# jcyk/gtos

Measured on AMD Instinct MI355X. Metric: graphs/sec training step (100-node AMR, batch 64), higher is better.
Workload: dtype bf16

## Files before the change

### gtos_amd/_lib.py

```python
import ctypes
import os
import threading

import torch

_HERE = os.path.dirname(os.path.abspath(__file__))
LIB_PATH = os.path.join(_HERE, "csrc", "libgtos_hip.so")
ABI_VERSION = 25

c_p, c_i, c_l, c_f, c_u64 = ctypes.c_void_p, ctypes.c_int, ctypes.c_int64, ctypes.c_float, ctypes.c_uint64

SIGNATURES = {
    "gtos_abi_version": [],
    "gtos_pathtrie_dev_workspace": [c_l, c_l, c_p],
    "gtos_pathtrie_dev_phase_a": [c_i, c_l, c_p, c_p, c_p, c_p, c_p, c_p, c_p, ctypes.c_size_t, c_p],
    "gtos_pathtrie_dev_phase_b": [c_l, c_l, c_i, c_i, c_i, c_i, c_p, c_p, c_p, c_p, c_p, ctypes.c_size_t, c_p],
    "gtos_relbatch_dev_workspace": [c_l, c_p],
    "gtos_relbatch_dev_phase_a": [c_p, c_p, c_p, ctypes.c_size_t, c_p],
    "gtos_relbatch_dev_phase_b": [c_p, c_l, c_p, c_p, ctypes.c_size_t, c_p],
    "gtos_relbatch_dev_all_count": [c_p, c_p, c_p, ctypes.c_size_t, c_p],
    "gtos_relbatch_dev_all_keys": [c_p, c_p, c_p, ctypes.c_size_t, c_p],
    "gtos_relbatch_dev_all_fill": [c_p, c_l, c_p, c_p, ctypes.c_size_t, c_p],
    "gtos_relindex_dev_workspace": [c_l, c_p],
    "gtos_relindex_dev_phase_a": [c_p, c_p, c_p, ctypes.c_size_t, c_p],
    "gtos_relindex_dev_phase_b": [c_p, c_l, c_p, c_p, ctypes.c_size_t, c_p],
    "gtos_gemm": [c_i, c_i, c_i, c_i, c_i, c_i, c_i, c_p, c_l, c_p, c_l, c_p, c_l, c_p, c_i, c_f, c_u64, c_i, c_i, c_p, c_l, c_p],
    "gtos_rel_attn_fwd": [c_i] * 7 + [c_p, c_l, c_p, c_l, c_p, c_l, c_p, c_p, c_p, c_p, c_f, c_f, c_u64, c_p, c_l, c_p, c_p, c_p],
    "gtos_rel_attn_bwd": [c_i] * 7 + [c_p, c_l, c_p, c_l, c_p, c_l, c_p, c_p, c_p, c_p, c_p, c_f, c_f, c_u64,
                                      c_p, c_l, c_p, c_p, c_p, c_l, c_p, c_p, c_l, c_p, c_l, c_p, c_l, c_p, c_l, c_p, c_p, c_p],
    "gtos_rel_attn_bwd_bank": [c_i] * 5 + [c_p, c_l, c_p, c_l, c_p, c_p, c_p, c_p, c_p, c_p, c_p, c_p, c_i, c_p, c_l, c_p, c_p],
    "gtos_ln_residual_fwd": [c_i, c_i, c_i, c_p, c_p, c_f, c_u64, c_p, c_p, c_f, c_p, c_p, c_p, c_p],
    "gtos_ln_residual_bwd": [c_i, c_i, c_i, c_p, c_p, c_p, c_f, c_u64, c_p, c_p, c_p, c_p, c_p, c_p, c_p, c_p],
    "gtos_ln_residual_fwd2": [c_i, c_i, c_i, c_i, c_i, c_p, c_p, c_f, c_u64, c_p, c_p, c_f, c_p, c_p, c_p, c_p, c_p],
    "gtos_ln_residual_bwd2": [c_i, c_i, c_i, c_i, c_i, c_p, c_p, c_p, c_p, c_f, c_u64, c_p, c_p, c_p, c_p, c_p, c_p, c_p, c_p],
    "gtos_relu_dropout_bwd": [c_i, c_l, c_p, c_p, c_f, c_p],
    "gtos_colsum": [c_i, c_i, c_i, c_l, c_p, c_p, c_p],
    "gtos_gru_cell_fwd": [c_i, c_i, c_i, c_p, c_p, c_p, c_p, c_l, c_p, c_p, c_f, c_u64, c_l, c_p],
    "gtos_gru_step_fwd": [c_i, c_i, c_p, c_l, c_i, c_p, c_p, c_p, c_p, c_p, c_p, c_p, c_p, c_p, c_p, c_p, c_p, c_i, c_p, c_l, c_p, c_p, c_p, c_l,
                          c_f, c_u64, c_l, c_p],
    "gtos_gru_step_bwd": [c_i, c_i, c_p, c_i, c_p, c_p, c_p, c_p, c_p, c_l, c_p, c_i, c_l, c_p, c_f, c_u64, c_l, c_p, c_i, c_p, c_p, c_p, c_i, c_p],
    "gtos_gru_step_bwd_fused": [c_i, c_i, c_p, c_i, c_p, c_p, c_p, c_p, c_p, c_l, c_p, c_i, c_l, c_p, c_f, c_u64, c_l, c_p, c_i, c_p, c_p, c_p, c_i,
# ... 115 lines not shown
```

### gtos_amd/csrc/gru_step.hip

```cpp
#include <cstdlib>
#include "common.h"

__attribute__((visibility("hidden"))) const void* gtos_zero_block();

#define GTOS_VMCNT(n) __builtin_amdgcn_s_waitcnt(0x0F70 | ((n) & 15) | (((n) >> 4) << 14))
#ifndef GTOS_RACE_DEMO
#define GTOS_VMCNT_LDS(n) __builtin_amdgcn_s_waitcnt(0x0070 | ((n) & 15) | (((n) >> 4) << 14))
#define GTOS_LGKM0() __builtin_amdgcn_s_waitcnt(0xc07f)
#else
#define GTOS_VMCNT_LDS(n) GTOS_VMCNT(n)
#define GTOS_LGKM0()
#endif

namespace {

constexpr int ROWB = 128, BK = 64, TM = 128, TC = 64, WROWS = 3 * TC;
constexpr int A_BYTES = TM * ROWB, B_BYTES = WROWS * ROWB;

__device__ __forceinline__ int swz(int row) { return ((row >> 1) & 7) ^ ((row >> 4) & 3); }
__device__ __forceinline__ int lds_off(int r, int c) { return r * ROWB + ((c ^ swz(r)) << 4); }

struct StepArgs {
    const bf16_t* x; int64_t ldx; int in_dim; const bf16_t* w_ih; const float* b_ih;
    const bf16_t* xg;
// ... 158 lines not shown
#pragma unroll
        for (int i = 0; i < 16; ++i) bhz[i] += t[i];
    }
    const float ks = a.p_drop > 0.f ? 1.f / (1.f - a.p_drop) : 1.f;
#pragma unroll
    for (int mt = 0; mt < 2; ++mt) {
        const int m = m0 + wave * 32 + mt * 16 + fr;
        if (m >= a.rows) continue;
        float xr[16], xz[16], xn[16], hp[16];
        if constexpr (HAS_X) {
            ldf16(a.b_ih + 2 * hs + cb, xn);
#pragma unroll
            for (int i = 0; i < 16; ++i) { xr[i] = 0.f; xz[i] = 0.f; xn[i] += acc[mt][8 + (i >> 2)][i & 3]; }
        } else if constexpr (MODE == 2) {
            const bf16_t* fp = a.gf + (int64_t)a.gf_idx[m] * 3 * hs + cb;
            const bf16_t* bp = a.gb + (int64_t)a.gb_idx[m] * 3 * hs + cb;
            float t[16];
            ld16(fp, xr); ld16(bp, t);
#pragma unroll
            for (int i = 0; i < 16; ++i) xr[i] += t[i];
            ld16(fp + hs, xz); ld16(bp + hs, t);
#pragma unroll
            for (int i = 0; i < 16; ++i) xz[i] += t[i];
            ld16(fp + 2 * hs, xn); ld16(bp + 2 * hs, t);
#pragma unroll
            for (int i = 0; i < 16; ++i) xn[i] += t[i];
            ldf16(a.b_ih + 2 * hs + cb, t);
#pragma unroll
            for (int i = 0; i < 16; ++i) xn[i] += t[i];
        } else {
            const bf16_t* xp = a.xg + (int64_t)m * 3 * hs + cb;
            ld16(xp, xr); ld16(xp + hs, xz); ld16(xp + 2 * hs, xn);
        }
        ld16(a.h_in + (int64_t)(a.h_idx ? a.h_idx[m] : m) * hs + cb, hp);
        float gr[16], gz[16], gn[16], hn[16], o[16];
#pragma unroll
        for (int i = 0; i < 16; ++i) {
            gr[i] = 1.f / (1.f + __expf(-(xr[i] + acc[mt][(i >> 2)][i & 3] + bhr[i])));
            gz[i] = 1.f / (1.f + __expf(-(xz[i] + acc[mt][4 + (i >> 2)][i & 3] + bhz[i])));
            hn[i] = acc[mt][GH * 4 + (i >> 2)][i & 3] + bhn[i];
            hn[i] = bf2f(f2bf(hn[i]));
            gn[i] = fast_tanh(xn[i] + gr[i] * hn[i]);
            o[i] = (1.f - gz[i]) * gn[i] + gz[i] * hp[i];
        }
        bf16_t* gp = a.gates + (int64_t)m * 4 * hs + cb;
        st16(gp, gr); st16(gp + hs, gz); st16(gp + 2 * hs, gn);
        st16(gp + 3 * hs, hn);
        bf16_t* hdst = m < a.n_out ? a.h_out + (int64_t)m * hs + cb
                                   : a.h_fin + (int64_t)(a.fin_idx ? a.fin_idx[m] : m) * a.ld_fin + cb;
        st16(hdst, o);
        if (a.y) {
            if (a.p_drop > 0.f) {
#pragma unroll
                for (int i = 0; i < 16; ++i)
                    o[i] = drop_keep(a.seed, (uint64_t)(a.drop_base + (int64_t)m * a.ldy + cb + i), a.p_drop) ? o[i] * ks : 0.f;
            }
            st16(a.y + (int64_t)m * a.ldy + cb, o);
        }
    }
}

template <int MODE>
__global__ __launch_bounds__(256, 2) void gru_step_fwd_kernel(StepArgs a) {
    if (a.p_drop > 0.f) a.seed = live_seed(a.seed);
    constexpr bool HAS_X = MODE == 1;
    constexpr int NG = HAS_X ? 4 : 3;
    constexpr int GH = HAS_X ? 3 : 2;
    __shared__ __attribute__((aligned(16))) char lds[A_BYTES + B_BYTES];
    char* As = lds;
    char* Bs = lds + A_BYTES;
    const int lane = threadIdx.x & 63, wave = __builtin_amdgcn_readfirstlane(threadIdx.x >> 6);
    const int fr = lane & 15, fq = lane >> 4;
    const int nC = a.hs / TC;
    const int xcd = blockIdx.x & 7, sq = blockIdx.x >> 3;
    const int m0 = ((sq / nC) * 8 + xcd) * TM, c0 = (sq % nC) * TC;
    if (m0 >= a.rows) return;
    const U128* Z = static_cast<const U128*>(a.zeros);

    f32x4_t acc[2][NG * 4];
#pragma unroll
    for (int i = 0; i < 2; ++i)
#pragma unroll
        for (int j = 0; j < NG * 4; ++j) acc[i][j] = f32x4_t{0.f, 0.f, 0.f, 0.f};

    if constexpr (HAS_X) {
        const RowSrc xs = row_src(a.x, a.ldx, a.rows, m0, wave, lane);
        const WSrc ws = w_src(a.in_dim, a.hs, c0, wave, lane);
        for (int k0 = 0; k0 < a.in_dim; k0 += BK) {
            dma_rows_at(xs, Z, k0, a.in_dim, As, wave);
            dma_weights_at(ws, a.w_ih, Z, k0, a.in_dim, Bs, wave);
            __syncthreads();
            mma_tile<NG, 2>(As, Bs, wave * 32, fr, fq, acc);
            __syncthreads();
        }
    }
    {
        const RowSrc hsrc = row_src(a.h_in, a.hs, a.rows, m0, wave, lane, a.h_idx);
        const WSrc ws = w_src(a.hs, a.hs, c0, wave, lane);
        for (int k0 = 0; k0 < a.hs; k0 += BK) {
            dma_rows_at(hsrc, Z, k0, a.hs, As, wave);
            dma_weights_at(ws, a.w_hh, Z, k0, a.hs, Bs, wave);
            __syncthreads();
            mma_tile<NG, GH>(As, Bs, wave * 32, fr, fq, acc);
            __syncthreads();
        }
    }

    step_cell<MODE>(a, acc, m0, c0, wave, fr, fq);
}


__global__ __launch_bounds__(512, 2) void gru_step_fwd_a2w3_kernel(StepArgs a) {
    constexpr int TMW = 256, AW = TMW * ROWB;
    if (a.p_drop > 0.f) a.seed = live_seed(a.seed);
    __shared__ __attribute__((aligned(16))) char sa0[AW];
    __shared__ __attribute__((aligned(16))) char sa1[AW];
    __shared__ __attribute__((aligned(16))) char sw0[B_BYTES];
    __shared__ __attribute__((aligned(16))) char sw1[B_BYTES];
    __shared__ __attribute__((aligned(16))) char sa2[AW];
    const int lane = threadIdx.x & 63, wave = __builtin_amdgcn_readfirstlane(threadIdx.x >> 6);
    const int fr = lane & 15, fq = lane >> 4;
    const int hs = a.hs, nC = hs / TC;
    const int xcd = blockIdx.x & 7, sq = blockIdx.x >> 3;
    const int m0 = ((sq / nC) * 8 + xcd) * TMW, c0 = (sq % nC) * TC;
    if (m0 >= a.rows) return;
    const int nkx = a.in_dim / BK, nk = nkx + hs / BK;
    uint32_t axo[4], aho[4], bxo[3], bho[3];
#pragma unroll
    for (int i = 0; i < 4; ++i) {
        const int rl = (i * 8 + wave) * 8 + (lane >> 3);
        const int r = min(m0 + rl, a.rows - 1) - m0;
        const uint32_t c = (uint32_t)(((lane & 7) ^ swz(rl)) << 4);
        axo[i] = (uint32_t)r * (uint32_t)(a.ldx * 2) + c;
        aho[i] = (uint32_t)r * (uint32_t)(hs * 2) + c;
    }
#pragma unroll
    for (int i = 0; i < 3; ++i) {
        const int rl = (i * 8 + wave) * 8 + (lane >> 3);
        const int g = rl >> 6, nt = (rl >> 4) & 3, q = (rl >> 2) & 3, e = rl & 3;
        const int wrow = g * hs + c0 + q * 16 + nt * 4 + e;
        const uint32_t c = (uint32_t)(((lane & 7) ^ swz(rl)) << 4);
        bxo[i] = (uint32_t)wrow * (uint32_t)(a.in_dim * 2) + c;
        bho[i] = (uint32_t)wrow * (uint32_t)(hs * 2) + c;
    }
    const char* Xb = reinterpret_cast<const char*>(a.x + (int64_t)m0 * a.ldx);
    const char* Hb = reinterpret_cast<const char*>(a.h_in + (int64_t)m0 * hs);
    const char* Wi = reinterpret_cast<const char*>(a.w_ih);
    const char* Wh = reinterpret_cast<const char*>(a.w_hh);

    f32x4_t acc[2][16];
#pragma unroll
    for (int i = 0; i < 2; ++i)
#pragma unroll
        for (int j = 0; j < 16; ++j) acc[i][j] = f32x4_t{0.f, 0.f, 0.f, 0.f};

#define GTOS_DMA1(src, dst)                                                                                                   \
    __builtin_amdgcn_global_load_lds((const __attribute__((address_space(1))) void*)(src),                                    \
                                     (__attribute__((address_space(3))) void*)(dst), 16, 0, 0)
#define GTOS_A2W3_DMA_A(slot, s_)                                                                                             \
    {                                                                                                                         \
        const int st_ = min((s_), nk - 1);                                                                                    \
        const bool px_ = st_ < nkx;                                                                                           \
        const char* ab_ = px_ ? Xb + st_ * ROWB : Hb + (st_ - nkx) * ROWB;                                                    \
        GTOS_DMA1(ab_ + (px_ ? axo[0] : aho[0]), (slot) + (0 * 8 + wave) * 1024);                                             \
        GTOS_DMA1(ab_ + (px_ ? axo[1] : aho[1]), (slot) + (1 * 8 + wave) * 1024);                                             \
        GTOS_DMA1(ab_ + (px_ ? axo[2] : aho[2]), (slot) + (2 * 8 + wave) * 1024);                                             \
        GTOS_DMA1(ab_ + (px_ ? axo[3] : aho[3]), (slot) + (3 * 8 + wave) * 1024);                                             \
    }
#define GTOS_A2W3_DMA_W(slot, s_)                                                                                             \
    {                                                                                                                         \
        const int st_ = min((s_), nk - 1);                                                                                    \
        const bool px_ = st_ < nkx;                                                                                           \
        const char* bb_ = px_ ? Wi + st_ * ROWB : Wh + (st_ - nkx) * ROWB;                                                    \
        GTOS_DMA1(bb_ + (px_ ? bxo[0] : bho[0]), (slot) + (0 * 8 + wave) * 1024);                                             \
        GTOS_DMA1(bb_ + (px_ ? bxo[1] : bho[1]), (slot) + (1 * 8 + wave) * 1024);                                             \
        GTOS_DMA1(bb_ + (px_ ? bxo[2] : bho[2]), (slot) + (2 * 8 + wave) * 1024);                                             \
    }
#define GTOS_A2W3_STEP(sa_, sw_, sa_n, sw_n, s_)                                                                              \
    {                                                                                                                         \
        GTOS_VMCNT_LDS(4);                                  \
        __builtin_amdgcn_s_barrier();                       \
        GTOS_A2W3_DMA_W(sw_n, (s_) + 1);                                                                                      \
        GTOS_A2W3_DMA_A(sa_n, (s_) + 2);                                                                                      \
        {                                                                                                                     \
            _Pragma("unroll") for (int ks = 0; ks < 2; ++ks) {                                                                \
                bf16x8_t fa[2], fb[12];                                                                                       \
                _Pragma("unroll") for (int mt = 0; mt < 2; ++mt)                                                              \
                    fa[mt] = *reinterpret_cast<const bf16x8_t*>((sa_) + lds_off(wave * 32 + mt * 16 + fr, ks * 4 + fq));      \
                _Pragma("unroll") for (int t = 0; t < 12; ++t)                                                                \
                    fb[t] = *reinterpret_cast<const bf16x8_t*>((sw_) + lds_off(t * 16 + fr, ks * 4 + fq));                    \
                _Pragma("unroll") for (int g = 0; g < 2; ++g)                                                                 \
                    _Pragma("unroll") for (int nt = 0; nt < 4; ++nt)                                                          \
                        _Pragma("unroll") for (int mt = 0; mt < 2; ++mt)                                                      \
                            acc[mt][g * 4 + nt] = __builtin_amdgcn_mfma_f32_16x16x32_bf16(fb[g * 4 + nt], fa[mt], acc[mt][g * 4 + nt], 0, 0, 0); \
                if ((s_) < nkx) {                                                                                             \
                    _Pragma("unroll") for (int nt = 0; nt < 4; ++nt)                                                          \
                        _Pragma("unroll") for (int mt = 0; mt < 2; ++mt)                                                      \
                            acc[mt][8 + nt] = __builtin_amdgcn_mfma_f32_16x16x32_bf16(fb[8 + nt], fa[mt], acc[mt][8 + nt], 0, 0, 0); \
                } else {                                                                                                      \
                    _Pragma("unroll") for (int nt = 0; nt < 4; ++nt)                                                          \
                        _Pragma("unroll") for (int mt = 0; mt < 2; ++mt)                                                      \
                            acc[mt][12 + nt] = __builtin_amdgcn_mfma_f32_16x16x32_bf16(fb[8 + nt], fa[mt], acc[mt][12 + nt], 0, 0, 0); \
                }                                                                                                             \
            }                                                                                                                 \
        }                                                                                                                     \
    }

    if (nk > 0) {
        GTOS_A2W3_DMA_A(sa0, 0);
        GTOS_A2W3_DMA_W(sw0, 0);
        GTOS_A2W3_DMA_A(sa1, 1);
    }
    for (int s = 0; s + 6 <= nk; s += 6) {
        GTOS_A2W3_STEP(sa0, sw0, sa2, sw1, s);
        GTOS_A2W3_STEP(sa1, sw1, sa0, sw0, s + 1);
        GTOS_A2W3_STEP(sa2, sw0, sa1, sw1, s + 2);
        GTOS_A2W3_STEP(sa0, sw1, sa2, sw0, s + 3);
        GTOS_A2W3_STEP(sa1, sw0, sa0, sw1, s + 4);
        GTOS_A2W3_STEP(sa2, sw1, sa1, sw0, s + 5);
    }
    GTOS_VMCNT(0);
#undef GTOS_A2W3_STEP
#undef GTOS_A2W3_DMA_W
#undef GTOS_A2W3_DMA_A
#undef GTOS_DMA1
    step_cell<1>(a, acc, m0, c0, wave, fr, fq);
}


struct Raw16 { uint4 a, b; };
__device__ __forceinline__ void unpack16(const Raw16& r, float (&v)[16]) {
    v[0] = lo_bf(r.a.x); v[1] = hi_bf(r.a.x); v[2] = lo_bf(r.a.y); v[3] = hi_bf(r.a.y);
    v[4] = lo_bf(r.a.z); v[5] = hi_bf(r.a.z); v[6] = lo_bf(r.a.w); v[7] = hi_bf(r.a.w);
    v[8] = lo_bf(r.b.x); v[9] = hi_bf(r.b.x); v[10] = lo_bf(r.b.y); v[11] = hi_bf(r.b.y);
    v[12] = lo_bf(r.b.z); v[13] = hi_bf(r.b.z); v[14] = lo_bf(r.b.w); v[15] = hi_bf(r.b.w);
}
__device__ __forceinline__ Raw16 ldraw16(const bf16_t* p) {
    Raw16 r;
    r.a = *reinterpret_cast<const uint4*>(p);
    r.b = *reinterpret_cast<const uint4*>(p + 8);
    return r;
}

constexpr int P_ROWS = 32;
constexpr int P_TM = 4 * P_ROWS;

template <int KT>
__global__ __launch_bounds__(256, 1) void gru_l1_fwd_persistent_kernel(StepArgs a, int n_workers) {
    extern __shared__ __attribute__((aligned(16))) char plds[];
    constexpr int HS = 64 * KT;
    constexpr int A_TILE = P_ROWS * ROWB;
    const int lane = threadIdx.x & 63, wave = __builtin_amdgcn_readfirstlane(threadIdx.x >> 6);
// ... 289 lines not shown
            __syncthreads();
#pragma unroll
            for (int ks = 0; ks < 2; ++ks) {
                bf16x8_t fa[2], fb[4];
#pragma unroll
                for (int mt = 0; mt < 2; ++mt) fa[mt] = *reinterpret_cast<const bf16x8_t*>(As + lds_off(wave * 32 + mt * 16 + fr, ks * 4 + fq));
#pragma unroll
                for (int nt = 0; nt < 4; ++nt) fb[nt] = *reinterpret_cast<const bf16x8_t*>(Bs + lds_off(nt * 16 + fr, ks * 4 + fq));
#pragma unroll
                for (int mt = 0; mt < 2; ++mt)
#pragma unroll
                    for (int nt = 0; nt < 4; ++nt)
                        acc[mt][nt] = __builtin_amdgcn_mfma_f32_16x16x32_bf16(fb[nt], fa[mt], acc[mt][nt], 0, 0, 0);
            }
            __syncthreads();
        }
    } else if (a.d4_prev && m0 < a.rows_prev) {
        kloop_a2<1, true>(a.d4_prev, 4 * (int64_t)hs, a.rows_prev, m0, a.wh_t, 3 * (int64_t)hs, c0, 1, hs, Z, As, lds_a1, Bs, acc, wave, lane);
    } else if (a.bias_part) {
        __syncthreads();
    }

    const int cb = c0 + fq * 16;
    const float ks = a.p_drop > 0.f ? 1.f / (1.f - a.p_drop) : 1.f;
#pragma unroll
    for (int mt = 0; mt < 2; ++mt) {
        const int m_raw = m0 + wave * 32 + mt * 16 + fr;
        const bool valid = m_raw < a.rows;
        const int m = valid ? m_raw : a.rows - 1;
        float gr[16], gz[16], gn[16], hn[16], hp[16], g[16];
        const bf16_t* gp = a.gates + (int64_t)m * 4 * hs + cb;
        ld16(gp, gr); ld16(gp + hs, gz); ld16(gp + 2 * hs, gn);
        ld16(gp + 3 * hs, hn);
        ld16(a.hprev + (int64_t)(a.hprev_idx ? a.hprev_idx[m] : m) * hs + cb, hp);
        float* dhp = static_cast<float*>(a.dh) + (int64_t)m * a.ld_dh + cb;
        bf16_t* dhb = static_cast<bf16_t*>(a.dh) + (int64_t)m * a.ld_dh + cb;
        if (a.sum_idx) {
            const int64_t sr = a.sum_idx[m];
            if (sr == a.zero_row) {
#pragma unroll
                for (int i = 0; i < 16; ++i) g[i] = 0.f;
            } else if (a.dh_bf16) ld16(static_cast<const bf16_t*>(a.dh_src) + sr * hs + cb, g);
            else ldf16(static_cast<const float*>(a.dh_src) + sr * hs + cb, g);
        } else if (a.dh_bf16) ld16(dhb, g); else ldf16(dhp, g);
#pragma unroll
        for (int i = 0; i < 16; ++i) g[i] += acc[mt][i >> 2][i & 3];
        if (a.dy) {
            float dyv[16];
            ld16(a.dy + (int64_t)m * a.ldy + cb, dyv);
#pragma unroll
            for (int i = 0; i < 16; ++i) {
                float t2 = dyv[i];
                if (a.p_drop > 0.f) t2 = drop_keep(a.seed, (uint64_t)(a.drop_base + (int64_t)m * a.ldy + cb + i), a.p_drop) ? t2 * ks : 0.f;
                g[i] += t2;
            }
        }
        float dr_[16], dz_[16], dn_[16], dhn[16];
#pragma unroll
        for (int i = 0; i < 16; ++i) {
            const float dn = g[i] * (1.f - gz[i]);
            const float dz = g[i] * (hp[i] - gn[i]);
            dn_[i] = dn * (1.f - gn[i] * gn[i]);
            dhn[i] = dn_[i] * gr[i];
            dr_[i] = dn_[i] * hn[i] * gr[i] * (1.f - gr[i]);
            dz_[i] = dz * gz[i] * (1.f - gz[i]);
            g[i] *= gz[i];
            if (!valid) { dn_[i] = 0.f; dhn[i] = 0.f; dr_[i] = 0.f; dz_[i] = 0.f; }
        }
        if (valid) {
            if (a.dh_bf16) {
                st16(dhb, g);
            } else {
#pragma unroll
                for (int i = 0; i < 4; ++i)
                    *reinterpret_cast<float4*>(dhp + i * 4) = make_float4(g[i * 4], g[i * 4 + 1], g[i * 4 + 2], g[i * 4 + 3]);
            }
            bf16_t* dp = a.d4 + (int64_t)m * 4 * hs + cb;
            st16(dp, dr_); st16(dp + hs, dz_); st16(dp + 2 * hs, dn_); st16(dp + 3 * hs, dhn);
            if (a.hp_out) st16(a.hp_out + (int64_t)m * hs + cb, hp);
        }
        if (a.bias_part) {
#pragma unroll
            for (int i = 0; i < 16; ++i) {
                const float t0 = row16_sum(bf2f(f2bf(dr_[i]))), t1 = row16_sum(bf2f(f2bf(dz_[i])));
                const float t2 = row16_sum(bf2f(f2bf(dn_[i]))), t3 = row16_sum(bf2f(f2bf(dhn[i])));
                if (fr == 0) {
                    atomicAdd(&btab[0 * TC + fq * 16 + i], t0); atomicAdd(&btab[1 * TC + fq * 16 + i], t1);
                    atomicAdd(&btab[2 * TC + fq * 16 + i], t2); atomicAdd(&btab[3 * TC + fq * 16 + i], t3);
                }
            }
        }
    }
    if (a.bias_part) {
        __syncthreads();
        const int q = threadIdx.x >> 6, ch = threadIdx.x & 63;
        float* dst = a.bias_part + (int64_t)(blockIdx.x % a.n_partials) * 4 * hs + q * hs + c0 + ch;
        atomicAdd(dst, btab[threadIdx.x]);
    }
}


}

extern "C" int gtos_gru_step_fwd(int rows, int hs, const void* x, int64_t ldx, int in_dim, const void* w_ih, const float* b_ih,
                                 const void* xg, const void* gf, const int* gf_idx, const void* gb, const int* gb_idx,
                                 const void* h_in, const int* h_idx, const void* w_hh, const float* b_hh,
                                 void* h_out, int n_out, void* h_fin, int64_t ld_fin, const int* fin_idx, void* gates, void* y, int64_t ldy,
                                 float p_drop, uint64_t seed, int64_t drop_base, void* stream) {
    if (rows <= 0) return 0;
    if (hs <= 0 || hs % TC) return -22;
    if (!h_in || !w_hh || !b_hh || !gates) return -23;
    if ((n_out > 0 && !h_out) || (n_out < rows && !h_fin)) return -23;
    if (h_fin && (ld_fin < hs || ld_fin % 8)) return -25;
    const int mode = x ? 1 : (gf ? 2 : 0);
    if (mode == 1) {
        if (!w_ih || !b_ih || in_dim <= 0 || in_dim % 8 || ldx % 8 || (uintptr_t)x % 16 || (uintptr_t)w_ih % 16) return -24;
    } else if (mode == 2) {
        if (!gb || !gf_idx || !gb_idx || !b_ih || (uintptr_t)gf % 16 || (uintptr_t)gb % 16) return -24;
    } else if (!xg || (uintptr_t)xg % 16) return -24;
    if ((uintptr_t)h_in % 16 || (uintptr_t)w_hh % 16 || (uintptr_t)gates % 16 || (uintptr_t)h_out % 16 || (uintptr_t)h_fin % 16 ||
        (uintptr_t)b_hh % 16 || (uintptr_t)b_ih % 16) return -25;
    if (y && ((uintptr_t)y % 16 || ldy % 8)) return -25;
    StepArgs a;
    a.x = (const bf16_t*)x; a.ldx = ldx; a.in_dim = in_dim; a.w_ih = (const bf16_t*)w_ih; a.b_ih = b_ih; a.xg = (const bf16_t*)xg;
    a.gf = (const bf16_t*)gf; a.gf_idx = gf_idx; a.gb = (const bf16_t*)gb; a.gb_idx = gb_idx;
    a.h_in = (const bf16_t*)h_in; a.h_idx = h_idx; a.w_hh = (const bf16_t*)w_hh; a.b_hh = b_hh;
    a.h_out = (bf16_t*)h_out; a.n_out = n_out; a.h_fin = (bf16_t*)h_fin; a.gates = (bf16_t*)gates; a.y = (bf16_t*)y; a.ldy = ldy;
    a.ld_fin = ld_fin; a.fin_idx = fin_idx;
    a.p_drop = p_drop; a.seed = seed; a.drop_base = drop_base; a.rows = rows; a.hs = hs;
    a.zeros = gtos_zero_block();
    if (!a.zeros) return -5;
    const long long nM = (rows + TM - 1) / TM, nC = hs / TC;
    const long long nblk = ((nM + 7) / 8) * 8 * nC;
    if (nblk > 0x7fffffffLL) return -6;
    hipStream_t s = static_cast<hipStream_t>(stream);
    if (mode == 2 && hs == 256 && !h_idx && !y && rows >= 16384) {
        constexpr int KT = 4;
        const size_t lds_bytes = (size_t)KT * B_BYTES + 4 * KT * P_ROWS * ROWB;
        static bool configured = false;
        if (!configured) {
            if (hipFuncSetAttribute(reinterpret_cast<const void*>(gru_l1_fwd_persistent_kernel<KT>),
                                    hipFuncAttributeMaxDynamicSharedMemorySize, (int)lds_bytes) != hipSuccess) return -7;
            configured = true;
        }
        const int n_cu = 256, n_workers = n_cu / KT;
        hipLaunchKernelGGL(gru_l1_fwd_persistent_kernel<KT>, dim3(n_cu), dim3(256), lds_bytes, s, a, n_workers);
        GTOS_CHECK_LAUNCH();
        return 0;
    }
    static const bool use_a2w3 = !(getenv("GTOS_GRU_FWD_A2W3") && getenv("GTOS_GRU_FWD_A2W3")[0] == '0');
    if (mode == 1 && use_a2w3 && rows >= 8192 && in_dim % 64 == 0 && (in_dim / 64 + hs / 64) % 6 == 0 && !h_idx && ldx < (1 << 20) &&
        (int64_t)3 * hs * (in_dim > hs ? in_dim : hs) * 2 < (1LL << 31)) {
        const long long nM8 = (rows + 255) / 256, nblk8 = ((nM8 + 7) / 8) * 8 * nC;
        hipLaunchKernelGGL(gru_step_fwd_a2w3_kernel, dim3((unsigned)nblk8), dim3(512), 0, s, a);
    }
    else if (mode == 1) hipLaunchKernelGGL(gru_step_fwd_kernel<1>, dim3((unsigned)nblk), dim3(256), 0, s, a);
    else if (mode == 2) hipLaunchKernelGGL(gru_step_fwd_kernel<2>, dim3((unsigned)nblk), dim3(256), 0, s, a);
    else hipLaunchKernelGGL(gru_step_fwd_kernel<0>, dim3((unsigned)nblk), dim3(256), 0, s, a);
    GTOS_CHECK_LAUNCH();
    return 0;
}

extern "C" int gtos_gru_step_bwd_fused(int rows, int hs, const void* d4_prev, int rows_prev, const void* w_hh_t,
                                       const void* gates, const void* hprev, const int* hprev_idx, const void* dy, int64_t ldy,
                                       void* dh, int dh_dtype, int64_t ld_dh, void* d4, float p_drop, uint64_t seed, int64_t drop_base,
                                       float* bias_partials, int n_partials, void* hprev_out, const int* sum_idx, const void* dh_src,
                                       int zero_row,
                                       const void* w_ih_t, void* dinp, int64_t ld_dinp, int n_in, int dinp_accumulate, float p_in,
                                       uint64_t seed_in, int64_t in_drop_base, void* stream) {
    const bool role_b = dinp != nullptr && d4_prev != nullptr && rows_prev > 0;
    if (rows <= 0 && !role_b) return 0;
    if (hs <= 0 || hs % TC) return -22;
    if (rows > 0) {
        if (!gates || !hprev || !dh || !d4 || (d4_prev && !w_hh_t)) return -23;
        if (sum_idx && (!dh_src || (uintptr_t)dh_src % 16)) return -23;
    }
    if (dinp && (!d4_prev || !w_ih_t || sum_idx)) return -23;
    if (dinp && (n_in <= 0 || n_in % TC || ld_dinp < n_in || ld_dinp % 8 || (uintptr_t)dinp % 16 || (uintptr_t)w_ih_t % 16)) return -27;
    if (bias_partials && n_partials < 1) return -26;
    if ((uintptr_t)d4_prev % 16 || (uintptr_t)w_hh_t % 16 || (uintptr_t)gates % 16 || (uintptr_t)hprev % 16 || (uintptr_t)dh % 16 ||
        (uintptr_t)d4 % 16 || (dy && ((uintptr_t)dy % 16 || ldy % 8)) || (rows > 0 && (ld_dh < hs || ld_dh % 8)) ||
        (uintptr_t)hprev_out % 16) return -25;
    StepBwdArgs a;
    a.d4_prev = (const bf16_t*)d4_prev; a.rows_prev = d4_prev ? rows_prev : 0; a.wh_t = (const bf16_t*)w_hh_t;
    a.gates = (const bf16_t*)gates; a.hprev = (const bf16_t*)hprev; a.hprev_idx = hprev_idx; a.dy = (const bf16_t*)dy; a.ldy = ldy;
    a.dh = dh; a.dh_bf16 = dh_dtype == GTOS_BF16; a.ld_dh = ld_dh; a.d4 = (bf16_t*)d4; a.bias_part = bias_partials; a.n_partials = n_partials;
    a.hp_out = (bf16_t*)hprev_out; a.sum_idx = sum_idx; a.dh_src = dh_src; a.zero_row = sum_idx ? zero_row : -1;
    a.wi_t = (const bf16_t*)w_ih_t; a.dinp = role_b ? (bf16_t*)dinp : nullptr; a.ld_dinp = ld_dinp; a.n_in = n_in; a.dinp_acc = dinp_accumulate;
    a.p_in = p_in; a.seed_in = seed_in; a.in_drop_base = in_drop_base;
    a.p_drop = p_drop; a.seed = seed; a.drop_base = drop_base; a.rows = rows > 0 ? rows : 0; a.hs = hs;
    a.zeros = gtos_zero_block();
    if (!a.zeros) return -5;
    const long long cover = role_b && rows_prev > a.rows ? rows_prev : a.rows;
    const long long nM = (cover + TM - 1) / TM, per = hs / TC + (role_b ? (n_in + 2 * TC - 1) / (2 * TC) : 0);
    const long long nblk = ((nM + 7) / 8) * 8 * per;
    if (nblk > 0x7fffffffLL) return -6;
    hipLaunchKernelGGL(gru_step_bwd_kernel<2>, dim3((unsigned)nblk), dim3(256), 0, static_cast<hipStream_t>(stream), a);
    GTOS_CHECK_LAUNCH();
    return 0;
}

extern "C" int gtos_gru_step_bwd(int rows, int hs, const void* d4_prev, int rows_prev, const void* w_hh_t,
                                 const void* gates, const void* hprev, const int* hprev_idx, const void* dy, int64_t ldy, void* dh, int dh_dtype,
                                 int64_t ld_dh, void* d4, float p_drop, uint64_t seed, int64_t drop_base, float* bias_partials,
                                 int n_partials, void* hprev_out, const int* sum_idx, const void* dh_src, int zero_row, void* stream) {
    return gtos_gru_step_bwd_fused(rows, hs, d4_prev, rows_prev, w_hh_t, gates, hprev, hprev_idx, dy, ldy, dh, dh_dtype, ld_dh, d4,
                                   p_drop, seed, drop_base, bias_partials, n_partials, hprev_out, sum_idx, dh_src, zero_row,
// ... 5 lines not shown
```

### gtos_amd/csrc/rowops.hip

```cpp
#include "common.h"

namespace {

constexpr int LN_MAXC = 2;

template <typename TX, typename TR, typename TY>
__global__ __launch_bounds__(256) void ln_fwd_kernel(int rows, int d, const TX* __restrict__ x, const TR* __restrict__ r,
                                                     float p_drop, uint64_t seed, const float* __restrict__ gamma,
                                                     const float* __restrict__ beta, float eps, TY* __restrict__ y, bf16_t* __restrict__ y2,
                                                     float* __restrict__ mean, float* __restrict__ rstd) {
    if (p_drop > 0.f) seed = live_seed(seed);
    const int lane = threadIdx.x & 63;
    const int row = blockIdx.x * 4 + (threadIdx.x >> 6);
    if (row >= rows) return;
    const float ks = p_drop > 0.f ? 1.f / (1.f - p_drop) : 1.f;
    float z[LN_MAXC][8];
    float s = 0.f;
#pragma unroll
    for (int cI = 0; cI < LN_MAXC; ++cI) {
        const int c = (cI * 64 + lane) * 8;
#pragma unroll
        for (int e = 0; e < 8; ++e) z[cI][e] = 0.f;
        if (c < d) {
            Vec8<TX>::load(x + (int64_t)row * d + c, z[cI]);
// ... 1087 lines not shown
                       (double)warmup_steps, (double)embed_dim, ctl);
    GTOS_CHECK_LAUNCH();
    return 0;
}

extern "C" int gtos_cast_f32_to_bf16(int64_t n, const float* src, void* dst, void* stream) {
    if (n <= 0) return 0;
    hipStream_t s = static_cast<hipStream_t>(stream);
    hipLaunchKernelGGL(cast_bf16_kernel, dim3(grid_for(n, 256 * 4)), dim3(256), 0, s, n, src, (bf16_t*)dst);
    GTOS_CHECK_LAUNCH();
    return 0;
}

extern "C" int gtos_transpose_batch_bf16(int n_mat, const int64_t* desc, const int* tile_start, int total_tiles, const void* src,
                                         void* dst, void* stream) {
    if (n_mat <= 0 || total_tiles <= 0) return 0;
    if (!desc || !tile_start || !src || !dst) return -23;
    hipLaunchKernelGGL(transpose_batch_kernel, dim3((unsigned)total_tiles), dim3(256), 0, static_cast<hipStream_t>(stream), n_mat, desc,
                       tile_start, (const bf16_t*)src, (bf16_t*)dst);
    GTOS_CHECK_LAUNCH();
    return 0;
}

extern "C" int gtos_set_seed_epoch(const void* epoch) {
    int rc = gtosi_gemm_set_seed_epoch(epoch);
    if (!rc) rc = gtosi_rel_attn_set_seed_epoch(epoch);
    if (!rc) rc = gtosi_attn_tile_set_seed_epoch(epoch);
    if (!rc) rc = gtosi_rowops_set_seed_epoch(epoch);
    if (!rc) rc = gtosi_gru_step_set_seed_epoch(epoch);
    if (!rc) rc = gtosi_tokenenc_set_seed_epoch(epoch);
    return rc;
}

extern "C" int gtos_abi_version(void) { return 25; }

GTOS_SEED_EPOCH_SETTER(rowops)
```

### gtos_amd/gru.py

```python
import contextlib
import os

import torch

from . import _lib
from ._lib import call, dt, ptr, stream
from .ops import (gemm, compute_weight, next_seed, weight_t, _grad_target, _splitk, side_stream as _side_stream, side_ok, defer_side_join, _Timed,
                  embed_bwd_workspace, _workspace, WORKSPACE_BYTES, note_memory)


def _cell_fwd(A, hs, xg, hg, h, y, y_off_elems, ldy, hprev, gates, p, seed, drop_base):
    yp = None if y is None else y.data_ptr() + y_off_elems * y.element_size()
    call("gtos_gru_cell_fwd", dt(xg), A, hs, ptr(xg), ptr(hg), ptr(h), yp, ldy, ptr(hprev), ptr(gates),
         float(p), seed, drop_base, stream())


N_BIAS_PARTIALS = 1024

FUSE = "x"
SIDE_STREAM = os.environ.get("GTOS_GRU_SIDE", "1") != "0"
SIDE_MIN_ROWS = 200000


def _step_fwd(A, hs, x, xg, h_in, wi, b_ih, wh, b_hh, h_out, n_out, h_fin, gates, y, y_off_elems, ldy, p, seed, drop_base,
              h_idx=None, gf=None, gf_idx=None, gb=None, gb_idx=None, fin_idx=None, tag=None):
    yp = None if y is None else y.data_ptr() + y_off_elems * y.element_size()
    need_bi = x is not None or gf is not None
    name = tag or "gru_step_fwd_%s" % ("x" if x is not None else ("tables" if gf is not None else "xg"))
    units = A if tag is None else A * 2 * (x.shape[1] + hs + 4 * hs + hs + (hs if y is not None else 0))
    with _Timed(name, detail=True, units=units):
        _step_fwd_call(A, hs, x, xg, h_in, wi, b_ih, wh, b_hh, h_out, n_out, h_fin, gates, yp, ldy, p, seed, drop_base,
                       h_idx, gf, gf_idx, gb, gb_idx, need_bi, fin_idx)


def _step_fwd_call(A, hs, x, xg, h_in, wi, b_ih, wh, b_hh, h_out, n_out, h_fin, gates, yp, ldy, p, seed, drop_base,
                   h_idx, gf, gf_idx, gb, gb_idx, need_bi, fin_idx=None):
    call("gtos_gru_step_fwd", A, hs, ptr(x), 0 if x is None else x.stride(0), 0 if x is None else x.shape[1],
         ptr(wi) if x is not None else None, ptr(b_ih) if need_bi else None, ptr(xg),
         ptr(gf), ptr(gf_idx), ptr(gb), ptr(gb_idx), ptr(h_in), ptr(h_idx), ptr(wh), ptr(b_hh),
         ptr(h_out), n_out, ptr(h_fin), hs if h_fin is None else h_fin.stride(0), ptr(fin_idx), ptr(gates), yp, ldy,
         float(p), seed, drop_base, stream())


def _step_bwd(A, hs, d4_prev, rows_prev, wh_t, gates, hprev, dy_ptr, ldy, dh, d4, p, seed, drop_base, bpart, hprev_idx=None, hp_out=None,
              sum_idx=None, dh_src=None, zero_row=-1):
    with _Timed("gru_step_bwd_%s" % ("trie" if hprev_idx is not None else "rows"), detail=True, units=A):
        call("gtos_gru_step_bwd", A, hs, ptr(d4_prev), rows_prev if d4_prev is not None else 0, ptr(wh_t), ptr(gates), ptr(hprev),
             ptr(hprev_idx), dy_ptr, ldy, ptr(dh), dt(dh), dh.stride(0), ptr(d4), float(p), seed, drop_base,
             ptr(bpart), N_BIAS_PARTIALS if bpart is not None else 0, ptr(hp_out), ptr(sum_idx), ptr(dh_src), int(zero_row), stream())


def _cell_bwd(A, hs, gates, hprev, dy, dy_off_elems, ldy, dh, dxg, dhg, p, seed, drop_base, bpart):
    dyp = None if dy is None else dy.data_ptr() + dy_off_elems * dy.element_size()
    call("gtos_gru_cell_bwd", dt(gates), A, hs, ptr(gates), ptr(hprev), dyp, ldy, ptr(dh), ptr(dxg), ptr(dhg),
         float(p), seed, drop_base, ptr(bpart), 0 if bpart is None else bpart.shape[0], stream())


class BiGRUFinalFn(torch.autograd.Function):

    @staticmethod
    def forward(ctx, x, batch_sizes, hs, num_layers, p_drop, *weights):
        L, R = len(batch_sizes), batch_sizes[0]
# ... 160 lines not shown
        return (dY if ctx.needs_input_grad[0] else None, None, None, None, None) + tuple(grads)


class PackPlan(object):

    def __init__(self, batch_sizes, order32, order64=None):
        self.batch_sizes = [int(a) for a in batch_sizes if a > 0]
        self.offs = [0]
        for a in self.batch_sizes:
            self.offs.append(self.offs[-1] + a)
        self.L, self.N = len(self.batch_sizes), self.offs[-1]
        self.order32 = order32
        self.order64 = order64 if order64 is not None else order32.to(torch.int64)
        self.offs_dev = torch.tensor(self.offs, dtype=torch.int32).to(order32.device, non_blocking=True)

    @staticmethod
    def of_trie(trie):
        plan = getattr(trie, "_pack_plan", None)
        if plan is None or plan.order32.device != trie.seq_order32.device:
            plan = trie._pack_plan = PackPlan(trie.batch_sizes, trie.seq_order32, trie.seq_order)
        return plan

    @staticmethod
    def of_lengths(lengths, max_len):
        sorted_len, order = torch.sort(lengths, descending=True, stable=True)
        bs = (sorted_len.unsqueeze(0) > torch.arange(max_len, device=lengths.device).unsqueeze(1)).sum(1).tolist()
        return PackPlan(bs, order.to(torch.int32), order)


def _step_bwd_fused(A, hs, d4_prev, rows_prev, wh_t, gates, hprev, dy_ptr, ldy, dh, d4, p, seed, drop_base, bpart,
                    wi_t=None, dinp=None, n_in=0, dinp_acc=False, p_in=0.0, seed_in=0, in_drop_base=0, tag="gru_step_bwd_packed"):
    rp = rows_prev if d4_prev is not None else 0
    both = min(A, rp) if dinp is not None else 0
    nbytes = 2 * (A * (4 * hs + hs + 2 * hs + 4 * hs + (hs if dy_ptr else 0)) + both * 4 * hs
                  + ((rp - both) * 3 * hs if dinp is not None else min(A, rp) * 3 * hs) + (rp * n_in * (2 if dinp_acc else 1) if dinp is not None else 0))
    with _Timed(tag, detail=True, units=nbytes):
        call("gtos_gru_step_bwd_fused", A, hs, ptr(d4_prev), rows_prev if d4_prev is not None else 0, ptr(wh_t), ptr(gates), ptr(hprev), None,
             dy_ptr, ldy, ptr(dh), 0 if dh is None else dt(dh), hs if dh is None else dh.stride(0), ptr(d4), float(p), seed, drop_base,
             ptr(bpart), N_BIAS_PARTIALS if bpart is not None else 0, None, None, None, -1,
             ptr(wi_t), ptr(dinp), 0 if dinp is None else dinp.stride(0), n_in, int(dinp_acc), float(p_in), seed_in, in_drop_base, stream())


D4_INPLACE = os.environ.get("GTOS_GRU_D4_INPLACE", "auto")
D4_INPLACE_MIN_BYTES = 8 << 30


class PackedPathGRUFn(torch.autograd.Function):

    @staticmethod
    def forward(ctx, bank, plan, table, dim_pad, p_embed, hs, p_layer, *weights):
        dev, dtp = table.device, torch.bfloat16
        bs, offs, L, N = plan.batch_sizes, plan.offs, plan.L, plan.N
        R = bank.shape[1]
        if L == 0 or R == 0:
            ctx.cfg = False
            return torch.zeros((R, 2 * hs), dtype=dtp, device=dev)
        V, dim = table.shape
        tab = table.detach()
        want_table = table.requires_grad and ctx.needs_input_grad[2]
        Vp = (V + 7) // 8 * 8
        X = torch.empty((N, dim_pad), dtype=dtp, device=dev)
        onehot = torch.empty((N, Vp), dtype=dtp, device=dev) if (want_table and V <= 256) else None
        tokens = torch.empty((N,), dtype=torch.int64, device=dev) if (want_table and V > 256) else None
        seed_e = next_seed() if p_embed > 0 else 0
        call("gtos_embed_packed_paths", dt(X), L, R, N, ptr(bank), ptr(plan.order32), ptr(plan.offs_dev), ptr(tab), dim, dim_pad, ptr(X),
             float(p_embed), seed_e, ptr(onehot), Vp, ptr(tokens), stream())
        fin = (torch.empty if bs[0] == R else torch.zeros)((R, 2 * hs), dtype=dtp, device=dev)
        park = [torch.empty((bs[0], hs), dtype=dtp, device=dev) for _ in (0, 1)]
        inp, saved = X, []
        for l in range(2):
            last = l == 1
            Y = None if last else torch.empty((N, 2 * hs), dtype=dtp, device=dev)
            seed = next_seed() if (p_layer > 0 and not last) else 0
            pl = p_layer if not last else 0.0
            layer_saved = []
            bufs = [(torch.empty((N, 4 * hs), dtype=dtp, device=dev), torch.empty((N, hs), dtype=dtp, device=dev)) for _ in (0, 1)]
            wts = []
            for direction in (0, 1):
                w_ih, w_hh, b_ih, b_hh = weights[l * 8 + direction * 4: l * 8 + direction * 4 + 4]
                wi, wh = compute_weight(w_ih, dtp), compute_weight(w_hh, dtp)
                if wi.shape[1] != inp.shape[1]:
                    wi = torch.nn.functional.pad(wi.detach(), (0, inp.shape[1] - wi.shape[1]))
                    wi_t = wi.t().contiguous()
                else:
                    wi_t = weight_t(w_ih, wi)
                wts.append((wi, wh, wi_t, weight_t(w_hh, wh), b_ih.detach(), b_hh.detach()))
            for direction in (0, 1):
                wi, wh, wi_t, wh_t, bi, bh = wts[direction]
                gates, hprev = bufs[direction]
                if direction == 0:
                    hprev[:bs[0]].zero_()
                else:
                    for t in range(L):
                        lo = bs[t + 1] if t + 1 < L else 0
                        if bs[t] > lo:
                            hprev[offs[t] + lo: offs[t] + bs[t]].zero_()
                h_fin = fin[:, direction * hs:(direction + 1) * hs] if last else park[direction]
                for t in (range(L) if direction == 0 else range(L - 1, -1, -1)):
                    A, off = bs[t], offs[t]
                    nxt = t + 1 if direction == 0 else t - 1
                    if 0 <= nxt < L:
                        h_out, n_out = hprev[offs[nxt]:], min(A, bs[nxt])
                    else:
                        h_out, n_out = None, 0
                    _step_fwd(A, hs, inp[off:off + A], None, hprev[off:off + A], wi, bi, wh, bh, h_out, n_out, h_fin, gates[off:off + A],
                              Y, off * 2 * hs + direction * hs, 2 * hs, pl, seed, off * 2 * hs + direction * hs,
                              fin_idx=plan.order32 if last else None, tag="gru_step_fwd_packed_l%d" % l)
                layer_saved.append((wi_t, wh_t, gates, hprev))
            saved.append((inp, seed, pl, layer_saved))
            inp = Y
        ctx.cfg = (plan, table, dim_pad, p_embed, seed_e, hs, weights, saved, onehot, tokens)
        return fin

    @staticmethod
    def backward(ctx, d_out):
        with _Timed("relation_gru_bwd"):
            return PackedPathGRUFn._backward(ctx, d_out)

    @staticmethod
    def _backward(ctx, d_out):
        if ctx.cfg is False:
            return (None,) * len(ctx.needs_input_grad)
        if ctx.cfg is None:
            raise RuntimeError("PackedPathGRUFn: backward called a second time -- the saved gates and states are released piece by piece "
                               "during the first (retain_graph is not supported on this path)")
        plan, table, dim_pad, p_embed, seed_e, hs, weights, saved, onehot, tokens = ctx.cfg
        bs, offs, L, N = plan.batch_sizes, plan.offs, plan.L, plan.N
        dev, dtp = d_out.device, torch.bfloat16
        dfin = d_out.to(dtp).index_select(0, plan.order64)
        grads = [None] * len(weights)
        for base in (8, 12, 0, 4):
            for slot in range(4):
                wt_ = weights[base + slot]
                if wt_.requires_grad and _grad_target(wt_) is None:
                    grads[base + slot] = torch.zeros(wt_.shape, dtype=torch.float32, device=dev)
        want_table = onehot is not None or tokens is not None
        main = torch.cuda.current_stream(dev)
        used_side, held = False, None
        dY = None
        dX = None
        saved = [list(e) for e in saved]
        ctx.cfg = None
        for l in (1, 0):
            inp, seed, pl, layer_saved = saved[l]
            saved[l] = None
            layer_saved = list(layer_saved)
            n_in = inp.shape[1]
            want_dinp = l == 1 or want_table
            d_in = torch.empty((N, n_in), dtype=dtp, device=dev) if want_dinp else None
            for direction in (0, 1):
                wi_t, wh_t, gates, hprev = layer_saved[direction]
                layer_saved[direction] = None
                base = l * 8 + direction * 4
                w_ih, w_hh, b_ih, b_hh = weights[base:base + 4]
                want_bias = b_ih.requires_grad or b_hh.requires_grad
                dh = dfin[:, direction * hs:(direction + 1) * hs] if l == 1 else torch.zeros((bs[0], hs), dtype=dtp, device=dev)
                in_place = D4_INPLACE == "1" or (D4_INPLACE != "0" and gates.numel() * gates.element_size() >= D4_INPLACE_MIN_BYTES)
                d4 = gates if in_place else torch.empty((N, 4 * hs), dtype=dtp, device=dev)
                note_memory(dev)
                bpart = torch.zeros((N_BIAS_PARTIALS, 4 * hs), dtype=torch.float32, device=dev) if want_bias else None
                rb = dict(wi_t=wi_t, n_in=n_in, dinp_acc=direction == 1, p_in=p_embed if l == 0 else 0.0,
                          seed_in=seed_e if l == 0 else 0) if want_dinp else None
                tag = "gru_step_bwd_packed_l%d" % l
                prev = None
                for t in (range(L - 1, -1, -1) if direction == 0 else range(L)):
                    A, off = bs[t], offs[t]
                    dyp = None if dY is None else dY.data_ptr() + (off * 2 * hs + direction * hs) * dY.element_size()
                    kw = {} if (rb is None or prev is None) else dict(rb, dinp=d_in[offs[prev]:], in_drop_base=offs[prev] * n_in)
                    _step_bwd_fused(A, hs, None if prev is None else d4[offs[prev]:], 0 if prev is None else bs[prev], wh_t,
                                    gates[off:off + A], hprev[off:off + A], dyp, 2 * hs, dh, d4[off:off + A], pl, seed,
                                    off * 2 * hs + direction * hs, bpart, tag=tag, **kw)
                    prev = t
                if rb is not None:
                    _step_bwd_fused(0, hs, d4[offs[prev]:], bs[prev], wh_t, None, None, None, 2 * hs, None, None, 0.0, 0, 0, None, tag=tag,
                                    **dict(rb, dinp=d_in[offs[prev]:], in_drop_base=offs[prev] * n_in))
                del gates
                side = _side_stream(dev) if (SIDE_STREAM and side_ok(dev) and N >= SIDE_MIN_ROWS) else main
                if held is not None:
                    main.wait_stream(_side_stream(dev))
                    held = None
                if side is not main:
                    side.wait_stream(main)
                    held = (d4, bpart, hprev, inp)
                with torch.cuda.stream(side):
                    tg_ih = _grad_target(w_ih) if w_ih.requires_grad else None
                    tg_hh = _grad_target(w_hh) if w_hh.requires_grad else None
                    tg_ih = grads[base] if (tg_ih is None and w_ih.requires_grad) else tg_ih
                    tg_hh = grads[base + 1] if (tg_hh is None and w_hh.requires_grad) else tg_hh
                    scr_ih = torch.zeros(w_ih.shape, dtype=torch.float32, device=dev) if tg_ih is None else tg_ih
                    scr_hh = torch.zeros(w_hh.shape, dtype=torch.float32, device=dev) if tg_hh is None else tg_hh
                    if (tg_ih is not None or tg_hh is not None) and w_ih.shape[1] % 4 == 0:
                        with _Timed("gru_dw_grouped_l%d" % l, detail=True, units=2 * N * 3 * hs * (w_ih.shape[1] + hs)):
                            ws = _workspace(dev)
                            call("gtos_gru_weight_grads", N, hs, n_in, w_ih.shape[1], ptr(d4), ptr(inp), inp.stride(0), ptr(hprev), hprev.stride(0),
                                 ptr(scr_ih), scr_ih.stride(0), ptr(scr_hh), scr_hh.stride(0), ptr(ws), ws.numel() * 4, stream())
                    elif tg_ih is not None or tg_hh is not None:
                        for (tg, dyv, xin, rows) in ((tg_hh, d4[:, :2 * hs], hprev, slice(0, 2 * hs)), (tg_hh, d4[:, 3 * hs:], hprev, slice(2 * hs, 3 * hs)),
                                                     (tg_ih, d4[:, :3 * hs], inp, slice(0, 3 * hs))):
                            if tg is None:
                                continue
                            sk = _splitk(rows.stop - rows.start, xin.shape[1], N)
                            if tg.shape[1] == xin.shape[1]:
                                gemm(dyv, xin, trans_a=True, out=tg[rows], accumulate=True, splitk=sk)
                            else:
# ... 354 lines not shown
```

Before: 844.2.

## Skip recurrent GEMM and state loads for rows starting from zero hidden state

GRU step kernels now accept a null previous hidden state: forward skips the h·W_hh GEMM K-loop and hidden loads, and backward treats the previous state as zero and drops the dh store. The packed-path driver splits each reverse-direction step into continuing rows and freshly started rows when the latter are numerous, and the first forward step passes no state. The layer-0 parking buffer for final states is removed. This adds extra kernel launches per split step and a remainder path in the pipelined K loop.

```diff
diff --git a/gtos_amd/_lib.py b/gtos_amd/_lib.py
--- a/gtos_amd/_lib.py
+++ b/gtos_amd/_lib.py
@@ -6,7 +6,7 @@
 
 _HERE = os.path.dirname(os.path.abspath(__file__))
 LIB_PATH = os.path.join(_HERE, "csrc", "libgtos_hip.so")
-ABI_VERSION = 25
+ABI_VERSION = 26
 
 c_p, c_i, c_l, c_f, c_u64 = ctypes.c_void_p, ctypes.c_int, ctypes.c_int64, ctypes.c_float, ctypes.c_uint64
 
diff --git a/gtos_amd/csrc/gru_step.hip b/gtos_amd/csrc/gru_step.hip
--- a/gtos_amd/csrc/gru_step.hip
+++ b/gtos_amd/csrc/gru_step.hip
@@ -214,7 +214,11 @@
             const bf16_t* xp = a.xg + (int64_t)m * 3 * hs + cb;
             ld16(xp, xr); ld16(xp + hs, xz); ld16(xp + 2 * hs, xn);
         }
-        ld16(a.h_in + (int64_t)(a.h_idx ? a.h_idx[m] : m) * hs + cb, hp);
+        if (a.h_in) ld16(a.h_in + (int64_t)(a.h_idx ? a.h_idx[m] : m) * hs + cb, hp);
+        else {
+#pragma unroll
+            for (int i = 0; i < 16; ++i) hp[i] = 0.f;
+        }
         float gr[16], gz[16], gn[16], hn[16], o[16];
 #pragma unroll
         for (int i = 0; i < 16; ++i) {
@@ -228,9 +232,8 @@
         bf16_t* gp = a.gates + (int64_t)m * 4 * hs + cb;
         st16(gp, gr); st16(gp + hs, gz); st16(gp + 2 * hs, gn);
         st16(gp + 3 * hs, hn);
-        bf16_t* hdst = m < a.n_out ? a.h_out + (int64_t)m * hs + cb
-                                   : a.h_fin + (int64_t)(a.fin_idx ? a.fin_idx[m] : m) * a.ld_fin + cb;
-        st16(hdst, o);
+        if (m < a.n_out) st16(a.h_out + (int64_t)m * hs + cb, o);
+        else if (a.h_fin) st16(a.h_fin + (int64_t)(a.fin_idx ? a.fin_idx[m] : m) * a.ld_fin + cb, o);
         if (a.y) {
             if (a.p_drop > 0.f) {
 #pragma unroll
@@ -276,7 +279,7 @@
             __syncthreads();
         }
     }
-    {
+    if (a.h_in) {
         const RowSrc hsrc = row_src(a.h_in, a.hs, a.rows, m0, wave, lane, a.h_idx);
         const WSrc ws = w_src(a.hs, a.hs, c0, wave, lane);
         for (int k0 = 0; k0 < a.hs; k0 += BK) {
@@ -306,7 +309,7 @@
     const int xcd = blockIdx.x & 7, sq = blockIdx.x >> 3;
     const int m0 = ((sq / nC) * 8 + xcd) * TMW, c0 = (sq % nC) * TC;
     if (m0 >= a.rows) return;
-    const int nkx = a.in_dim / BK, nk = nkx + hs / BK;
+    const int nkx = a.in_dim / BK, nk = a.h_in ? nkx + hs / BK : nkx;
     uint32_t axo[4], aho[4], bxo[3], bho[3];
 #pragma unroll
     for (int i = 0; i < 4; ++i) {
@@ -326,7 +329,7 @@
         bho[i] = (uint32_t)wrow * (uint32_t)(hs * 2) + c;
     }
     const char* Xb = reinterpret_cast<const char*>(a.x + (int64_t)m0 * a.ldx);
-    const char* Hb = reinterpret_cast<const char*>(a.h_in + (int64_t)m0 * hs);
+    const char* Hb = a.h_in ? reinterpret_cast<const char*>(a.h_in + (int64_t)m0 * hs) : Xb;
     const char* Wi = reinterpret_cast<const char*>(a.w_ih);
     const char* Wh = reinterpret_cast<const char*>(a.w_hh);
 
@@ -393,13 +396,27 @@
         GTOS_A2W3_DMA_W(sw0, 0);
         GTOS_A2W3_DMA_A(sa1, 1);
     }
-    for (int s = 0; s + 6 <= nk; s += 6) {
+    int s = 0;
+    for (; s + 6 <= nk; s += 6) {
         GTOS_A2W3_STEP(sa0, sw0, sa2, sw1, s);
         GTOS_A2W3_STEP(sa1, sw1, sa0, sw0, s + 1);
         GTOS_A2W3_STEP(sa2, sw0, sa1, sw1, s + 2);
         GTOS_A2W3_STEP(sa0, sw1, sa2, sw0, s + 3);
         GTOS_A2W3_STEP(sa1, sw0, sa0, sw1, s + 4);
         GTOS_A2W3_STEP(sa2, sw1, sa1, sw0, s + 5);
+    }
+    if (s < nk) {
+        GTOS_A2W3_STEP(sa0, sw0, sa2, sw1, s);
+        if (s + 1 < nk) {
+            GTOS_A2W3_STEP(sa1, sw1, sa0, sw0, s + 1);
+            if (s + 2 < nk) {
+                GTOS_A2W3_STEP(sa2, sw0, sa1, sw1, s + 2);
+                if (s + 3 < nk) {
+                    GTOS_A2W3_STEP(sa0, sw1, sa2, sw0, s + 3);
+                    if (s + 4 < nk) GTOS_A2W3_STEP(sa1, sw0, sa0, sw1, s + 4);
+                }
+            }
+        }
     }
     GTOS_VMCNT(0);
 #undef GTOS_A2W3_STEP
@@ -755,7 +772,11 @@
         const bf16_t* gp = a.gates + (int64_t)m * 4 * hs + cb;
         ld16(gp, gr); ld16(gp + hs, gz); ld16(gp + 2 * hs, gn);
         ld16(gp + 3 * hs, hn);
-        ld16(a.hprev + (int64_t)(a.hprev_idx ? a.hprev_idx[m] : m) * hs + cb, hp);
+        if (a.hprev) ld16(a.hprev + (int64_t)(a.hprev_idx ? a.hprev_idx[m] : m) * hs + cb, hp);
+        else {
+#pragma unroll
+            for (int i = 0; i < 16; ++i) hp[i] = 0.f;
+        }
         float* dhp = static_cast<float*>(a.dh) + (int64_t)m * a.ld_dh + cb;
         bf16_t* dhb = static_cast<bf16_t*>(a.dh) + (int64_t)m * a.ld_dh + cb;
         if (a.sum_idx) {
@@ -791,7 +812,8 @@
             if (!valid) { dn_[i] = 0.f; dhn[i] = 0.f; dr_[i] = 0.f; dz_[i] = 0.f; }
         }
         if (valid) {
-            if (a.dh_bf16) {
+            if (!a.hprev) {
+            } else if (a.dh_bf16) {
                 st16(dhb, g);
             } else {
 #pragma unroll
@@ -832,8 +854,9 @@
                                  float p_drop, uint64_t seed, int64_t drop_base, void* stream) {
     if (rows <= 0) return 0;
     if (hs <= 0 || hs % TC) return -22;
-    if (!h_in || !w_hh || !b_hh || !gates) return -23;
-    if ((n_out > 0 && !h_out) || (n_out < rows && !h_fin)) return -23;
+    if (!w_hh || !b_hh || !gates) return -23;
+    if (!h_in && (!x || h_idx)) return -23;
+    if (n_out > 0 && !h_out) return -23;
     if (h_fin && (ld_fin < hs || ld_fin % 8)) return -25;
     const int mode = x ? 1 : (gf ? 2 : 0);
     if (mode == 1) {
@@ -895,7 +918,8 @@
     if (rows <= 0 && !role_b) return 0;
     if (hs <= 0 || hs % TC) return -22;
     if (rows > 0) {
-        if (!gates || !hprev || !dh || !d4 || (d4_prev && !w_hh_t)) return -23;
+        if (!gates || !dh || !d4 || (d4_prev && !w_hh_t)) return -23;
+        if (!hprev && (sum_idx || hprev_idx)) return -23;
         if (sum_idx && (!dh_src || (uintptr_t)dh_src % 16)) return -23;
     }
     if (dinp && (!d4_prev || !w_ih_t || sum_idx)) return -23;
diff --git a/gtos_amd/csrc/rowops.hip b/gtos_amd/csrc/rowops.hip
--- a/gtos_amd/csrc/rowops.hip
+++ b/gtos_amd/csrc/rowops.hip
@@ -1143,6 +1143,6 @@
     return rc;
 }
 
-extern "C" int gtos_abi_version(void) { return 25; }
+extern "C" int gtos_abi_version(void) { return 26; }
 
 GTOS_SEED_EPOCH_SETTER(rowops)
diff --git a/gtos_amd/gru.py b/gtos_amd/gru.py
--- a/gtos_amd/gru.py
+++ b/gtos_amd/gru.py
@@ -27,7 +27,8 @@
     yp = None if y is None else y.data_ptr() + y_off_elems * y.element_size()
     need_bi = x is not None or gf is not None
     name = tag or "gru_step_fwd_%s" % ("x" if x is not None else ("tables" if gf is not None else "xg"))
-    units = A if tag is None else A * 2 * (x.shape[1] + hs + 4 * hs + hs + (hs if y is not None else 0))
+    stored = A if h_fin is not None else min(A, n_out)
+    units = A if tag is None else 2 * (A * (x.shape[1] + (hs if h_in is not None else 0) + 4 * hs + (hs if y is not None else 0)) + stored * hs)
     with _Timed(name, detail=True, units=units):
         _step_fwd_call(A, hs, x, xg, h_in, wi, b_ih, wh, b_hh, h_out, n_out, h_fin, gates, yp, ldy, p, seed, drop_base,
                        h_idx, gf, gf_idx, gb, gb_idx, need_bi, fin_idx)
@@ -254,7 +255,8 @@
                     wi_t=None, dinp=None, n_in=0, dinp_acc=False, p_in=0.0, seed_in=0, in_drop_base=0, tag="gru_step_bwd_packed"):
     rp = rows_prev if d4_prev is not None else 0
     both = min(A, rp) if dinp is not None else 0
-    nbytes = 2 * (A * (4 * hs + hs + 2 * hs + 4 * hs + (hs if dy_ptr else 0)) + both * 4 * hs
+    state = (hs + 2 * hs) if hprev is not None else hs
+    nbytes = 2 * (A * (4 * hs + state + 4 * hs + (hs if dy_ptr else 0)) + both * 4 * hs
                   + ((rp - both) * 3 * hs if dinp is not None else min(A, rp) * 3 * hs) + (rp * n_in * (2 if dinp_acc else 1) if dinp is not None else 0))
     with _Timed(tag, detail=True, units=nbytes):
         call("gtos_gru_step_bwd_fused", A, hs, ptr(d4_prev), rows_prev if d4_prev is not None else 0, ptr(wh_t), ptr(gates), ptr(hprev), None,
@@ -265,6 +267,21 @@
 
 D4_INPLACE = os.environ.get("GTOS_GRU_D4_INPLACE", "auto")
 D4_INPLACE_MIN_BYTES = 8 << 30
+
+
+START_SPLIT_MIN_ROWS = 8192
+
+
+def _step_parts(bs, t, direction):
+    A = bs[t]
+    if direction == 0:
+        return [(0, A, t == 0)]
+    s = bs[t + 1] if t + 1 < len(bs) else 0
+    if s == 0:
+        return [(0, A, True)]
+    if A - s >= START_SPLIT_MIN_ROWS:
+        return [(0, s, False), (s, A, True)]
+    return [(0, A, False)]
 
 
 class PackedPathGRUFn(torch.autograd.Function):
@@ -288,7 +305,6 @@
         call("gtos_embed_packed_paths", dt(X), L, R, N, ptr(bank), ptr(plan.order32), ptr(plan.offs_dev), ptr(tab), dim, dim_pad, ptr(X),
              float(p_embed), seed_e, ptr(onehot), Vp, ptr(tokens), stream())
         fin = (torch.empty if bs[0] == R else torch.zeros)((R, 2 * hs), dtype=dtp, device=dev)
-        park = [torch.empty((bs[0], hs), dtype=dtp, device=dev) for _ in (0, 1)]
         inp, saved = X, []
         for l in range(2):
             last = l == 1
@@ -317,17 +333,17 @@
                         lo = bs[t + 1] if t + 1 < L else 0
                         if bs[t] > lo:
                             hprev[offs[t] + lo: offs[t] + bs[t]].zero_()
-                h_fin = fin[:, direction * hs:(direction + 1) * hs] if last else park[direction]
+                h_fin = fin[:, direction * hs:(direction + 1) * hs] if last else None
                 for t in (range(L) if direction == 0 else range(L - 1, -1, -1)):
                     A, off = bs[t], offs[t]
                     nxt = t + 1 if direction == 0 else t - 1
-                    if 0 <= nxt < L:
-                        h_out, n_out = hprev[offs[nxt]:], min(A, bs[nxt])
-                    else:
-                        h_out, n_out = None, 0
-                    _step_fwd(A, hs, inp[off:off + A], None, hprev[off:off + A], wi, bi, wh, bh, h_out, n_out, h_fin, gates[off:off + A],
-                              Y, off * 2 * hs + direction * hs, 2 * hs, pl, seed, off * 2 * hs + direction * hs,
-                              fin_idx=plan.order32 if last else None, tag="gru_step_fwd_packed_l%d" % l)
+                    n_cont = min(A, bs[nxt]) if 0 <= nxt < L else 0
+                    for (r0, r1, zero) in _step_parts(bs, t, direction):
+                        lo, n_out = off + r0, max(0, min(n_cont, r1) - r0)
+                        _step_fwd(r1 - r0, hs, inp[lo:off + r1], None, None if zero else hprev[lo:off + r1], wi, bi, wh, bh,
+                                  hprev[offs[nxt] + r0:] if n_out > 0 else None, n_out, h_fin, gates[lo:off + r1],
+                                  Y, lo * 2 * hs + direction * hs, 2 * hs, pl, seed, lo * 2 * hs + direction * hs,
+                                  fin_idx=plan.order32[r0:] if last else None, tag="gru_step_fwd_packed_l%d" % l)
                 layer_saved.append((wi_t, wh_t, gates, hprev))
             saved.append((inp, seed, pl, layer_saved))
             inp = Y
@@ -387,11 +403,15 @@
                 prev = None
                 for t in (range(L - 1, -1, -1) if direction == 0 else range(L)):
                     A, off = bs[t], offs[t]
-                    dyp = None if dY is None else dY.data_ptr() + (off * 2 * hs + direction * hs) * dY.element_size()
-                    kw = {} if (rb is None or prev is None) else dict(rb, dinp=d_in[offs[prev]:], in_drop_base=offs[prev] * n_in)
-                    _step_bwd_fused(A, hs, None if prev is None else d4[offs[prev]:], 0 if prev is None else bs[prev], wh_t,
-                                    gates[off:off + A], hprev[off:off + A], dyp, 2 * hs, dh, d4[off:off + A], pl, seed,
-                                    off * 2 * hs + direction * hs, bpart, tag=tag, **kw)
+                    parts = _step_parts(bs, t, direction)
+                    for (r0, r1, zero) in parts:
+                        rp = 0 if prev is None else max(0, (bs[prev] if r1 == A else min(bs[prev], r1)) - r0)
+                        lo, po = off + r0, (0 if prev is None else offs[prev] + r0)
+                        dyp = None if dY is None else dY.data_ptr() + (lo * 2 * hs + direction * hs) * dY.element_size()
+                        kw = {} if (rb is None or rp == 0) else dict(rb, dinp=d_in[po:], in_drop_base=po * n_in)
+                        _step_bwd_fused(r1 - r0, hs, None if rp == 0 else d4[po:], rp, wh_t,
+                                        gates[lo:off + r1], None if zero else hprev[lo:off + r1], dyp, 2 * hs, dh[r0:], d4[lo:off + r1], pl, seed,
+                                        lo * 2 * hs + direction * hs, bpart, tag=tag, **kw)
                     prev = t
                 if rb is not None:
                     _step_bwd_fused(0, hs, d4[offs[prev]:], bs[prev], wh_t, None, None, None, 2 * hs, None, None, 0.0, 0, 0, None, tag=tag,
```

After: 847.6, median of 6. No clear change (+0.4%).
